# JasperSnoek/spearmint

Hardware: NVIDIA H100
Metric: EI candidates/sec (higher is better)
Workload: dtype f32

## Files before the change

### spearmint_b200/chooser/GPEIOptChooserB200.py

```python
import time

import numpy as np
import numpy.random as npr
import scipy.optimize as spo

from spearmint_b200 import chains, util
from spearmint_b200.chooser._gp import GPChooser, GPPrior, read_state, write_state, write_stats
from spearmint_b200.locker import log


def init(expt_dir, arg_string):
    args = util.unpack_args(arg_string)
    return GPEIOptChooserB200(expt_dir, **args)


class GPEIOptChooserB200(GPChooser):
    prior = GPPrior(max_ls=2, amp2_prior_on_std=True)

    def __init__(self, expt_dir, covar="Matern52", mcmc_iters=10, pending_samples=100, noiseless=False, burnin=100,
                 grid_subset=20, use_multiprocessing=True, device=None, refine_dtype="float64", state_name=None,
                 backend=None, grid_dtype="float32", mcmc_chains=1):
        GPChooser.__init__(self, expt_dir, covar, mcmc_iters, pending_samples, noiseless, state_name, device, backend,
                           refine_dtype, grid_dtype)
        self.mcmc_chains = int(mcmc_chains)
        if self.mcmc_chains < 1:
            raise ValueError("mcmc_chains must be at least 1, got %d" % self.mcmc_chains)
        if self.mcmc_iters > 0 and self.mcmc_iters % self.mcmc_chains:
            raise ValueError("mcmc_iters (%d) must be a multiple of mcmc_chains (%d)" % (self.mcmc_iters,
                                                                                       self.mcmc_chains))
        self.chains = None
        self.burnin = int(burnin)
        self.needs_burnin = True
        self.grid_subset = int(grid_subset)
        self.hyper_samples = []
        self.use_multiprocessing = bool(int(use_multiprocessing))
        self.stats = {}

    def dump_hypers(self):
        state = {"dims": self.D, "ls": self.ls, "amp2": self.amp2, "noise": self.noise,
                 "hyper_samples": self.hyper_samples, "mean": self.mean}
        if self.chains is not None:
            state["chains"] = [c.state() for c in self.chains]
        write_state(self.locker, self.state_pkl, state)
        write_stats(self.stats_file, self.hyper_samples)

    def _load_state(self, state):
        self._load_hypers(state)
        self.hyper_samples = state["hyper_samples"]
        self.needs_burnin = False
        if self.mcmc_chains > 1 and "chains" in state:
            if len(state["chains"]) != self.mcmc_chains:
                raise ValueError("the state pickle holds %d chains, mcmc_chains is %d" % (len(state["chains"]),
                                                                                        self.mcmc_chains))
            self.chains = [chains.Chain.from_state(c, st) for c, st in enumerate(state["chains"])]

    def generate_stats_html(self):
        state = read_state(self.state_pkl)
        if state is None:
            return "Chooser not yet ready to display output"
        self._load_state(state)
        mean_mean = np.mean(np.vstack([h[0] for h in self.hyper_samples]))
        mean_noise = np.mean(np.vstack([h[1] for h in self.hyper_samples]))
        mean_ls = np.mean(np.vstack([h[3][np.newaxis, :] for h in self.hyper_samples]), 0)
        try:
            output = ('<br /><span class="label label-info">Estimated mean:</span> ' + str(mean_mean) +
                      '<br /><span class="label label-info">Estimated noise:</span> ' + str(mean_noise) +
                      '<br /><br /><span class="label label-info">Inverse parameter sensitivity' +
                      ' - Gaussian Process length scales</span><br /><br />' +
                      '<div id="lschart"></div><script type="text/javascript">' +
                      'var lsdata = [' + ','.join(['%.2f' % i for i in mean_ls]) + '];')
        except Exception:
            return "Chooser not yet ready to display output."
        output += 'bar_chart("#lschart", lsdata, ' + str(self.prior.max_ls) + ');' + '</script>'
        return output

    def _real_init(self, dims, values):
        self.randomstate = npr.get_state()
        state = self._read_state()
        if state is not None:
            self._load_state(state)
        else:
            self._init_hypers(dims, values)
            self.hyper_samples.append((self.mean, self.noise, self.amp2, self.ls))

    def next(self, grid, values, durations, candidates, pending, complete):
        if complete.shape[0] < 2:
            return int(candidates[0])
        if self.D == -1:
            self._real_init(grid.shape[1], values[complete])

        comp = grid[complete, :]
        cand = grid[candidates, :]
        pend = grid[pending, :]
        vals = values[complete]
        numcand = cand.shape[0]

        best_comp = np.argmin(vals)
        cand2 = np.vstack((np.random.randn(10, comp.shape[1]) * 0.001 + comp[best_comp, :], cand))

        if self.mcmc_iters <= 0:
            raise NotImplementedError("mcmc_iters=0 (ML-II hyper-parameters) is broken in the reference "
                                      "(GPEIOptChooser.py:316-318) and not provided here")

        t_phase = [time.perf_counter()]
        phase_ms = {}

        def lap(name):
            t_phase.append(time.perf_counter())
            phase_ms[name] = phase_ms.get(name, 0.0) + 1e3 * (t_phase[-1] - t_phase[-2])

        if self.mcmc_chains > 1:
            self._sample_chains(comp, vals)
        else:
            self._loglik = self.backend.loglik(self.covar, comp, vals)
            if self.needs_burnin:
                for mcmc_iter in range(self.burnin):
                    self.sample_hypers(comp, vals)
                    log("BURN %d/%d] mean: %.2f  amp: %.2f noise: %.4f  min_ls: %.4f  max_ls: %.4f"
                        % (mcmc_iter + 1, self.burnin, self.mean, np.sqrt(self.amp2), self.noise,
                           np.min(self.ls), np.max(self.ls)))
                self.needs_burnin = False

            self.hyper_samples = []
            for mcmc_iter in range(self.mcmc_iters):
                self.sample_hypers(comp, vals)
                log("%d/%d] mean: %.2f  amp: %.2f  noise: %.4f min_ls: %.4f  max_ls: %.4f"
                    % (mcmc_iter + 1, self.mcmc_iters, self.mean, np.sqrt(self.amp2), self.noise,
                       np.min(self.ls), np.max(self.ls)))
            self.dump_hypers()
            self.stats["loglik_evals"] = getattr(self._loglik, "calls", None)
            self.stats["loglik_batches"] = getattr(self._loglik, "launch_batches", None)
            self._loglik = None
        lap("mcmc")

        b = [(0, 1)] * cand.shape[1]

        state = self._grid_state(comp, pend, vals)
        inds = self.backend.top_mean_ei(state, cand2, min(self.grid_subset, cand2.shape[0]))
        cand2 = cand2[inds, :]
        lap("grid_pass_1")

        ctx = self._refine_context(comp, pend, vals)
        for i in range(cand2.shape[0]):
            log("Optimizing candidate %d/%d" % (i + 1, cand2.shape[0]))
            ret = spo.fmin_l_bfgs_b(ctx.value_grad, cand2[i, :].flatten(), bounds=b)
            cand2[i, :] = ret[0]
        cand = np.vstack((cand, cand2))
        self.stats["refine_evals"] = getattr(ctx, "evals", None)
        del ctx
        lap("refine")

        best_cand = int(self.backend.top_mean_ei(state, cand, 1)[-1])
        self._set_current(self.hyper_samples[-1])
        lap("grid_pass_2")
        self.stats["phase_ms"] = phase_ms

        if best_cand >= numcand:
            return (int(numcand), cand[best_cand, :])
        return int(candidates[best_cand])

    def _fantasy_normals(self, pend):
        if pend.shape[0] == 0:
            return None
        npr.set_state(self.randomstate)
        return npr.randn(pend.shape[0], self.pending_samples)

    def _grid_state(self, comp, pend, vals):
        return self.backend.grid_state(self.covar, self.hyper_samples, comp, pend, vals, self._fantasy_normals(pend))

    def _refine_context(self, comp, pend, vals):
        return self.backend.refine_context(self.covar, self.hyper_samples, comp, pend, vals,
                                           self._fantasy_normals(pend))

    def _set_current(self, hyper):
        self.mean, self.noise, self.amp2, self.ls = hyper[0], hyper[1], hyper[2], hyper[3]

    def ei_over_hypers(self, comp, pend, cand, vals):
        hs = self.hyper_samples[:self.mcmc_iters]
        st = self.backend.grid_state(self.covar, hs, comp, pend, vals, self._fantasy_normals(pend))
        out = self.backend.ei_matrix(st, cand)
        self._set_current(hs[-1])
        return out

    def compute_ei(self, comp, pend, cand, vals):
        hs = [(self.mean, self.noise, self.amp2, self.ls)]
        st = self.backend.grid_state(self.covar, hs, comp, pend, vals, self._fantasy_normals(pend))
        return self.backend.ei_matrix(st, cand)[:, 0]

    def grad_optimize_ei_over_hypers(self, cand, comp, pend, vals, compute_grad=True):
        f, g = self._refine_context(comp, pend, vals).value_grad(cand)
        return (f, g) if compute_grad else f

    def _sample_chains(self, comp, vals):
        K = self.mcmc_chains
        if self.chains is None:
            self.chains = chains.Chain.seeded(K, (self.mean, self.noise, self.amp2, self.ls))
        ll = self.backend.loglik(self.covar, comp, vals, chains=K)
        self.hyper_samples, rounds = chains.sample(self.chains, self.prior, ll, vals, self.noiseless, self.burnin,
                                                   self.mcmc_iters // K)
        self._set_current(self.hyper_samples[-1])
        self.needs_burnin = False
        self.dump_hypers()
        self.stats["loglik_evals"] = getattr(ll, "calls", None)
        self.stats["loglik_batches"] = getattr(ll, "launch_batches", None)
        self.stats["chain_rounds"] = rounds

    def sample_hypers(self, comp, vals):
        ll = self._ll(comp, vals)
        if self.noiseless:
            self.noise = 1e-3
        self.mean, self.amp2, self.noise = self.prior.joint(ll, self.mean, self.amp2, self.noise, self.ls, vals,
                                                            self.noiseless)
        self.ls = self.prior.length_scales(ll, self.mean, self.noise, self.amp2, self.ls)
        self.hyper_samples.append((self.mean, self.noise, self.amp2, self.ls))
```

### spearmint_b200/csrc/potrf_ll.cu

```cuda
#include <cuda_runtime.h>

#include <algorithm>
#include <cstdlib>
#include <map>
#include <tuple>

#include "common.cuh"
#include "diag.cuh"

namespace smk {
int num_sms();
namespace ll {

constexpr int NB = 128;
constexpr int KC = 16;
constexpr int LDS = 20;
constexpr int STAGES = 3;

constexpr int WD = NB * 32;

__device__ __forceinline__ void pdl_wait() { asm volatile("griddepcontrol.wait;" ::: "memory"); }
__device__ __forceinline__ void pdl_trigger() { asm volatile("griddepcontrol.launch_dependents;" ::: "memory"); }

__global__ void __launch_bounds__(256) diag_kernel(int ld, int jb, double* __restrict__ A, long a_stride,
                                                    double* __restrict__ W, long w_stride, int* __restrict__ info) {
  extern __shared__ __align__(16) unsigned char smem_raw[];
  const int s = blockIdx.x;
  double* Ab = A + (long)s * a_stride + (long)jb * NB * ld + (long)jb * NB;
  pdl_wait();
  diag_factor_block<double, NB>(Ab, ld, W + (long)s * w_stride + (long)jb * WD, info ? info + s : nullptr, jb * NB,
                                reinterpret_cast<double*>(smem_raw), true);
}

__global__ void __launch_bounds__(256) panel_kernel(int ld, int jb, int row_blk0, double* __restrict__ A, long a_stride,
                                                     const double* __restrict__ W, long w_stride) {
  extern __shared__ __align__(16) unsigned char smem_raw[];
  const int s = blockIdx.z;
  double* As = A + (long)s * a_stride;
  pdl_wait();
  panel_sub_block<double, NB>(As + ((long)row_blk0 * NB + (long)blockIdx.x * 32) * ld + (long)jb * NB, ld,
                              As + (long)jb * NB * ld + (long)jb * NB, W + (long)s * w_stride + (long)jb * WD, nullptr,
                              nullptr, reinterpret_cast<double*>(smem_raw), true);
}

__device__ __forceinline__ void cp_async16(void* dst, const void* src) {
  asm volatile("cp.async.cg.shared.global [%0], [%1], 16;" ::"r"((unsigned)__cvta_generic_to_shared(dst)), "l"(src) : "memory");
}
__device__ __forceinline__ void cp_async_commit() { asm volatile("cp.async.commit_group;" ::: "memory"); }
template <int N> __device__ __forceinline__ void cp_async_wait() { asm volatile("cp.async.wait_group %0;" ::"n"(N) : "memory"); }

__device__ __forceinline__ void dmma(double (&c)[2], double a, double b) { dmma_884(c, a, b); }

struct GemmArgs {
  const double* A; const double* B; double* C;
  long a_stride, b_stride, c_stride;
  int lda, ldb, ldc, K;
  int row0, col0;
  int brow0;
  int sub, tri;
  int persist, nt, batch;
};

template <int BM, int ST>
__global__ void __launch_bounds__(256) dgemm_nt_kernel(GemmArgs g) {
  constexpr int WM = BM / 32, WN = 8 / WM;
  constexpr int WTN = 128 / WN;
  constexpr int NT = WTN / 8;
  extern __shared__ __align__(16) unsigned char smem_raw[];
  double* As = reinterpret_cast<double*>(smem_raw);
  double* Bs = As + ST * BM * LDS;

  const int tid = threadIdx.x, warp = tid >> 5, lane = tid & 31;
  const int wm = warp / WN, wn = warp % WN, gq = lane >> 2, t4 = lane & 3;
  const int ntri = g.nt * (g.nt + 1) / 2;
  const long items = g.persist ? (long)g.batch * ntri : 1;
  for (long item = g.persist ? blockIdx.x : 0; item < items; item += gridDim.x) {
    int bx = blockIdx.x, by = blockIdx.y, bz = blockIdx.z;
    if (g.persist) {
      bz = (int)(item / ntri);
      const int e = (int)(item - (long)bz * ntri);
      bx = (int)((sqrtf(8.f * (float)e + 1.f) - 1.f) * 0.5f);
      while (bx * (bx + 1) / 2 > e) --bx;
      while ((bx + 1) * (bx + 2) / 2 <= e) ++bx;
      by = e - bx * (bx + 1) / 2;
    }
    const int r0 = g.row0 + bx * BM, c0 = g.col0 + by * 128;
    if (g.tri && c0 > r0 + BM - 1) continue;
    const double* A = g.A + (long)bz * g.a_stride + (long)r0 * g.lda;
    const double* B = g.B + (long)bz * g.b_stride + (long)(g.brow0 + by * 128) * g.ldb;
    double* C = g.C + (long)bz * g.c_stride + (long)r0 * g.ldc + c0;

    auto load_stage = [&](int st, int k0) {
#pragma unroll
      for (int q = 0; q < BM * 8 / 256; ++q) {
        const int ch = tid + q * 256, row = ch >> 3, pc = ch & 7;
        cp_async16(As + ((size_t)st * BM + row) * LDS + pc * 2, A + (long)row * g.lda + k0 + pc * 2);
      }
#pragma unroll
      for (int q = 0; q < 4; ++q) {
        const int ch = tid + q * 256, row = ch >> 3, pc = ch & 7;
        cp_async16(Bs + ((size_t)st * 128 + row) * LDS + pc * 2, B + (long)row * g.ldb + k0 + pc * 2);
      }
    };

    double acc[4][NT][2];
#pragma unroll
    for (int mi = 0; mi < 4; ++mi)
#pragma unroll
      for (int ni = 0; ni < NT; ++ni) { acc[mi][ni][0] = 0.0; acc[mi][ni][1] = 0.0; }

    const int nk = g.K / KC;
#pragma unroll
    for (int s = 0; s < ST - 1; ++s) {
      if (s < nk) load_stage(s, s * KC);
      cp_async_commit();
    }
    for (int kt = 0; kt < nk; ++kt) {
      cp_async_wait<ST - 2>();
      __syncthreads();
      if (kt + ST - 1 < nk) load_stage((kt + ST - 1) % ST, (kt + ST - 1) * KC);
      cp_async_commit();
      const double* as = As + ((size_t)(kt % ST) * BM + wm * 32 + gq) * LDS + t4;
      const double* bs = Bs + ((size_t)(kt % ST) * 128 + wn * WTN + gq) * LDS + t4;
#pragma unroll
      for (int kk = 0; kk < KC; kk += 4) {
        double af[4], bf[NT];
#pragma unroll
        for (int mi = 0; mi < 4; ++mi) af[mi] = as[mi * 8 * LDS + kk];
#pragma unroll
        for (int ni = 0; ni < NT; ++ni) bf[ni] = bs[ni * 8 * LDS + kk];
#pragma unroll
        for (int mi = 0; mi < 4; ++mi)
#pragma unroll
          for (int ni = 0; ni < NT; ++ni) dmma(acc[mi][ni], af[mi], bf[ni]);
      }
    }
    cp_async_wait<0>();
    __syncthreads();

#pragma unroll
    for (int mi = 0; mi < 4; ++mi)
#pragma unroll
      for (int ni = 0; ni < NT; ++ni) {
        double2* cp = reinterpret_cast<double2*>(C + (long)(wm * 32 + mi * 8 + gq) * g.ldc + wn * WTN + ni * 8 + t4 * 2);
        double2 v;
        if (g.sub) { v = *cp; v.x -= acc[mi][ni][0]; v.y -= acc[mi][ni][1]; }
        else { v.x = acc[mi][ni][0]; v.y = acc[mi][ni][1]; }
        *cp = v;
      }
  }
}

constexpr int DBU_MAXK = 256;
__global__ void __launch_bounds__(256) diag_block_update_kernel(int ld, int b, int k0, int K, double* __restrict__ A, long a_stride) {
  extern __shared__ __align__(16) unsigned char smem_raw[];
  const int LD = K + 4;
  double* Ar = reinterpret_cast<double*>(smem_raw);
  double* Br = Ar + 32 * LD;
  int ti = 0, e = blockIdx.x;
  while ((ti + 1) * (ti + 2) / 2 <= e) ++ti;
  const int tj = e - ti * (ti + 1) / 2;
  double* As = A + (long)blockIdx.y * a_stride;
  const double* pa = As + ((long)b * NB + ti * 32) * ld + k0;
  const double* pb = As + ((long)b * NB + tj * 32) * ld + k0;
  const int tid = threadIdx.x, warp = tid >> 5, lane = tid & 31, gq = lane >> 2, t4 = lane & 3;
  pdl_wait();
  pdl_trigger();
  const int cpr = K / 2;
  for (int ch = tid; ch < 32 * cpr; ch += 256) {
    const int row = ch / cpr, pc = ch - row * cpr;
    cp_async16(Ar + row * LD + pc * 2, pa + (long)row * ld + pc * 2);
    cp_async16(Br + row * LD + pc * 2, pb + (long)row * ld + pc * 2);
  }
  cp_async_commit();
  cp_async_wait<0>();
  __syncthreads();
  double* Ct = As + ((long)b * NB + ti * 32) * ld + (long)b * NB + tj * 32;
#pragma unroll
  for (int u = 0; u < 2; ++u) {
    const int t = 2 * warp + u, r0 = (t >> 2) * 8, c0 = (t & 3) * 8;
    const double* ap = Ar + (r0 + gq) * LD + t4;
    const double* bp = Br + (c0 + gq) * LD + t4;
    double c[2][2] = {{0.0, 0.0}, {0.0, 0.0}};
#pragma unroll 8
    for (int k = 0; k < K; k += 8) {
      dmma(c[0], ap[k], bp[k]);
      dmma(c[1], ap[k + 4], bp[k + 4]);
    }
    double2* cp = reinterpret_cast<double2*>(Ct + (long)(r0 + gq) * ld + c0 + t4 * 2);
    double2 v = *cp;
    v.x -= c[0][0] + c[1][0];
    v.y -= c[0][1] + c[1][1];
    *cp = v;
  }
}

template <int BM>
static void launch_gemm(const GemmArgs& g, int tiles_m, int tiles_n, int S, cudaStream_t st) {
  constexpr int ST = STAGES;
  const size_t smem = sizeof(double) * ST * (BM + 128) * LDS;
  static bool attr = false;
  if (!attr) {
    cudaFuncSetAttribute(dgemm_nt_kernel<BM, ST>, cudaFuncAttributeMaxDynamicSharedMemorySize, (int)smem);
    attr = true;
  }
  dgemm_nt_kernel<BM, ST><<<dim3(tiles_m, tiles_n, S), 256, smem, st>>>(g);
}

template <int ST>
static void launch_gemm_background_st(GemmArgs g, int nt, int S, int ctas, cudaStream_t st) {
  const size_t smem = sizeof(double) * ST * (128 + 128) * LDS;
  static bool attr = false;
  if (!attr) {
    cudaFuncSetAttribute(dgemm_nt_kernel<128, ST>, cudaFuncAttributeMaxDynamicSharedMemorySize, (int)smem);
    attr = true;
  }
  g.persist = 1; g.nt = nt; g.batch = S;
  const long items = (long)S * nt * (nt + 1) / 2;
  dgemm_nt_kernel<128, ST><<<(unsigned)std::min<long>(items, ctas), 256, smem, st>>>(g);
}
static void launch_gemm_background(const GemmArgs& g, int nt, int S, int ctas, cudaStream_t st) {
  static int stages = -1;
  if (stages < 0) { const char* e = getenv("SMK_LL_BG_STAGES"); stages = (e && e[0] == '3') ? 3 : 2; }
  if (stages == 3) launch_gemm_background_st<3>(g, nt, S, ctas, st);
  else launch_gemm_background_st<2>(g, nt, S, ctas, st);
}

template <typename... KArgs, typename... Args>
static void launch_spine(void (*kern)(KArgs...), dim3 grid, size_t smem, cudaStream_t st, Args... args) {
  static int pdl = -1;
  if (pdl < 0) { const char* e = getenv("SMK_LL_PDL"); pdl = (e && e[0] == '0') ? 0 : 1; }
  cudaLaunchConfig_t cfg = {};
  cfg.gridDim = grid; cfg.blockDim = dim3(256); cfg.dynamicSmemBytes = smem; cfg.stream = st;
  cudaLaunchAttribute at[1];
  at[0].id = cudaLaunchAttributeProgrammaticStreamSerialization;
  at[0].val.programmaticStreamSerializationAllowed = 1;
  cfg.attrs = at; cfg.numAttrs = pdl ? 1 : 0;
  cudaLaunchKernelEx(&cfg, kern, KArgs(args)...);
}

struct Streams {
  cudaStream_t main = nullptr, near = nullptr, side = nullptr;
  cudaEvent_t diag0 = nullptr, diag1 = nullptr, head0 = nullptr, col = nullptr, la = nullptr, larest = nullptr, larest2 = nullptr, panel = nullptr, rest = nullptr,
              join_near = nullptr, join_side = nullptr;
};
static Streams& streams() {
  static Streams s;
  if (!s.main) {
    int lo = 0, hi = 0;
    cudaDeviceGetStreamPriorityRange(&lo, &hi);
    cudaStreamCreateWithPriority(&s.main, cudaStreamNonBlocking, hi);
    cudaStreamCreateWithPriority(&s.near, cudaStreamNonBlocking, hi < lo ? hi + 1 : hi);
    cudaStreamCreateWithPriority(&s.side, cudaStreamNonBlocking, lo);
    for (cudaEvent_t* e : {&s.diag0, &s.diag1, &s.head0, &s.col, &s.la, &s.larest, &s.larest2, &s.panel, &s.rest, &s.join_near, &s.join_side})
      cudaEventCreateWithFlags(e, cudaEventDisableTiming);
  }
  return s;
}

static int enqueue(int Npad, int S, double* A, double* W, int* info, Streams& ss) {
  const int nblk = Npad / NB;
  const long as = (long)Npad * Npad, ws = (long)nblk * WD;
  const size_t dsm = DiagSmem<double, NB>::bytes, psm = PanelSmem<double, NB>::bytes;
  static bool attr = false;
  if (!attr) {
    cudaFuncSetAttribute(diag_kernel, cudaFuncAttributeMaxDynamicSharedMemorySize, (int)dsm);
    cudaFuncSetAttribute(panel_kernel, cudaFuncAttributeMaxDynamicSharedMemorySize, (int)psm);
    cudaFuncSetAttribute(diag_block_update_kernel, cudaFuncAttributeMaxDynamicSharedMemorySize,
                         (int)(sizeof(double) * 2 * 32 * (DBU_MAXK + 4)));
    attr = true;
  }
  const size_t dbu_smem = sizeof(double) * 2 * 32 * (DBU_MAXK + 4);
  cudaStream_t m = ss.main, nr = ss.near, sd = ss.side;
  auto gemm_args = [&](int jcol, int K, int row_blk, int col_blk, int tri) {
    GemmArgs g{};
    g.A = A + (long)jcol * NB; g.lda = Npad; g.a_stride = as;
    g.B = A + (long)jcol * NB; g.ldb = Npad; g.b_stride = as; g.brow0 = col_blk * NB;
    g.C = A; g.ldc = Npad; g.c_stride = as;
    g.K = K; g.row0 = row_blk * NB; g.col0 = col_blk * NB; g.sub = 1; g.tri = tri;
    return g;
  };
  bool pend_col = false, pend_la = false, pend_la2 = false, side_used = false, near_used = false;
  const int reserve = std::min(24, std::max(8, 10 * S + 2));
  const int bg_ctas = std::max(num_sms() - reserve, 1);
  const double* Wc = W;
  for (int j = 0; j < nblk; j += 2) {
    launch_spine(diag_kernel, dim3(S), dsm, m, Npad, j, A, as, W, ws, info);
    count_launch();
    const int rem = nblk - j - 1;
    if (rem <= 0) break;
    if (pend_la) { cudaStreamWaitEvent(m, ss.larest, 0); pend_la = false; }
    if (rem > 1) {
      cudaEventRecord(ss.diag0, m);
      cudaStreamWaitEvent(nr, ss.diag0, 0);
      panel_kernel<<<dim3((rem - 1) * 4, 1, S), 256, psm, nr>>>(Npad, j, j + 2, A, as, Wc, ws);
      count_launch();
      near_used = true;
    }
    launch_spine(panel_kernel, dim3(4, 1, S), psm, m, Npad, j, j + 1, A, as, Wc, ws);
    if (pend_la2) { cudaStreamWaitEvent(m, ss.larest2, 0); pend_la2 = false; }
    launch_spine(diag_block_update_kernel, dim3(10, S), dbu_smem, m, Npad, j + 1, j * NB, NB, A, as);
    count_launch(2);
    if (rem > 1) {
      cudaEventRecord(ss.head0, m);
      cudaStreamWaitEvent(nr, ss.head0, 0);
      launch_gemm<32>(gemm_args(j, NB, j + 2, j + 1, 0), (rem - 1) * 4, 1, S, nr);
      cudaEventRecord(ss.col, nr);
      count_launch();
      pend_col = true;
    }
    launch_spine(diag_kernel, dim3(S), dsm, m, Npad, j + 1, A, as, W, ws, info);
    count_launch();
    const int rem2 = nblk - j - 2;
    if (rem2 <= 0) break;
    if (rem2 > 1) {
      cudaEventRecord(ss.diag1, m);
      cudaStreamWaitEvent(nr, ss.diag1, 0);
      panel_kernel<<<dim3((rem2 - 1) * 4, 1, S), 256, psm, nr>>>(Npad, j + 1, j + 3, A, as, Wc, ws);
      cudaEventRecord(ss.panel, nr);
      count_launch();
    }
    if (pend_col) { cudaStreamWaitEvent(m, ss.col, 0); pend_col = false; }
    launch_spine(panel_kernel, dim3(4, 1, S), psm, m, Npad, j + 1, j + 2, A, as, Wc, ws);
    count_launch();
    if (side_used) cudaStreamWaitEvent(m, ss.rest, 0);
    launch_spine(diag_block_update_kernel, dim3(10, S), dbu_smem, m, Npad, j + 2, j * NB, 2 * NB, A, as);
    count_launch();
    if (rem2 > 1) {
      cudaEventRecord(ss.la, m);
      cudaStreamWaitEvent(nr, ss.la, 0);
      launch_gemm<32>(gemm_args(j, 2 * NB, j + 3, j + 2, 0), (rem2 - 1) * 4, 1, S, nr);
      cudaEventRecord(ss.larest, nr);
      launch_gemm<32>(gemm_args(j, 2 * NB, j + 3, j + 3, 1), (rem2 - 1) * 4, 1, S, nr);
      cudaEventRecord(ss.larest2, nr);
      count_launch(2);
      pend_la = pend_la2 = true;
    }
    if (rem2 > 2) {
      cudaStreamWaitEvent(sd, ss.panel, 0);
      launch_gemm_background(gemm_args(j, 2 * NB, j + 4, j + 4, 1), rem2 - 2, S, bg_ctas, sd);
      cudaEventRecord(ss.rest, sd);
      count_launch();
      side_used = true;
    }
  }
  if (near_used) {
    cudaEventRecord(ss.join_near, nr);
    cudaStreamWaitEvent(m, ss.join_near, 0);
  }
  if (side_used) {
    cudaEventRecord(ss.join_side, sd);
    cudaStreamWaitEvent(m, ss.join_side, 0);
  }
  return 0;
}

}

static std::map<cudaGraphExec_t, int>& launches_per_graph() {
  static std::map<cudaGraphExec_t, int> m;
  return m;
}

size_t potrf_ll_workspace_bytes(int Npad, int S) { return (size_t)S * (Npad / ll::NB) * ll::WD * sizeof(double); }

int potrf_ll_f64(int Npad, int S, double* A, double* W, int* info, int use_graph, cudaStream_t st) {
  if (Npad <= 0 || Npad % ll::NB) return -1;
  if (S <= 0) return -2;
  if (!A || !W || !info) return -3;
  ll::Streams& ss = ll::streams();
  static cudaEvent_t ev_in = nullptr, ev_out = nullptr;
  if (!ev_in) {
    cudaEventCreateWithFlags(&ev_in, cudaEventDisableTiming);
    cudaEventCreateWithFlags(&ev_out, cudaEventDisableTiming);
  }
  cudaMemsetAsync(info, 0, sizeof(int) * S, st);
  if (!use_graph) {
    cudaEventRecord(ev_in, st);
// ... 41 lines not shown
```

### spearmint_b200/engine.py

```python
import ctypes as C
import os

import numpy as np
import scipy.stats as sps
import torch

from . import _lib
from ._lib import KINDS, check, fn, ptr

JITTER = 1e-6
CONSTRAINT_NOISE = 1e-3


def _ceil(x, m):
    return ((x + m - 1) // m) * m


class HyperBatch(object):

    def __init__(self, hyper_samples, kind, device, dtype):
        S = len(hyper_samples)
        D = len(np.atleast_1d(hyper_samples[0][3]))
        mean = np.array([h[0] for h in hyper_samples], dtype=np.float64)
        noise = np.array([h[1] for h in hyper_samples], dtype=np.float64)
        amp2 = np.array([h[2] for h in hyper_samples], dtype=np.float64)
        ls = np.vstack([np.atleast_1d(h[3]) for h in hyper_samples]).astype(np.float64)
        if kind == "SE":
            ls = np.ones_like(ls)
        host = np.concatenate([mean, noise, amp2, (1.0 / ls).ravel()])
        dev = torch.from_numpy(host).to(device=device, dtype=dtype, non_blocking=False)
        self.S, self.D = S, D
        self.mean, self.noise, self.amp2 = dev[:S], dev[S:2 * S], dev[2 * S:3 * S]
        self.inv_ls = dev[3 * S:].view(S, D)
        self.host_mean, self.host_noise, self.host_amp2, self.host_ls = mean, noise, amp2, ls
        self.nbytes = host.size * (8 if dtype == torch.float64 else 4)

    def slice(self, a, b):
        o = object.__new__(HyperBatch)
        o.S, o.D = b - a, self.D
        o.mean, o.noise, o.amp2, o.inv_ls = self.mean[a:b], self.noise[a:b], self.amp2[a:b], self.inv_ls[a:b]
        o.host_mean, o.host_noise = self.host_mean[a:b], self.host_noise[a:b]
        o.host_amp2, o.host_ls = self.host_amp2[a:b], self.host_ls[a:b]
        o.nbytes = 0
        return o


class Factor(object):

    def __init__(self, eng, kind, X, hb, L=None, winv=None, info=None, factor_impl=None):
        self.eng, self.kind, self.hb = eng, kind, hb
        self.factor_impl = factor_impl or eng.factor_impl
        self.X = X
        self.N, self.D = X.shape
        self.Npad = _ceil(self.N, 128)
        S, dt, dev = hb.S, eng.dtype, eng.device
        NB = eng.NB
        self._owned = []
        self.L = L if L is not None else self._take((S, self.Npad, self.Npad))
        self.winv = winv if winv is not None else self._take((S, self.Npad // NB, NB, NB))
        self.info = info if info is not None else torch.zeros((S,), dtype=torch.int32, device=dev)
        st = eng.stream()
        check(fn("smk_cov_build", dt)(KINDS[kind], self.N, self.N, self.D, S, ptr(X), None, ptr(hb.inv_ls),
                                      ptr(hb.amp2), ptr(hb.noise), ptr(self.L), self.Npad, st), "cov_build")
        if self.factor_impl == "tc" and dt == torch.float32 and self.Npad >= 256:
            L = _lib.lib()
            nb = 2 * S * self.Npad * self.Npad * 4
            ws = eng.take((nb,), torch.uint8)
            if eng.fused_inverse:
                Np = L.smk_tc_np(self.N)
                hi = self._take((S, Np, Np), torch.float32)
                lo = self._take((S, Np, Np), torch.float32)
                nt = L.smk_trtri_tc_workspace_bytes(self.Npad, Np, S)
                wt = eng.take((nt,), torch.uint8)
                check(L.smk_potrf_trtri_tc_f32(self.Npad, Np, S, ptr(self.L), ptr(self.winv), ptr(self.info), ptr(ws), nb,
                                               ptr(hi), ptr(lo), ptr(wt), nt, st), "potrf_trtri_tc")
                eng.give(ws, wt)
                self._linv = (hi, lo, Np)
            else:
                eng.give(ws)
                check(L.smk_potrf_lower_batched_tc_f32(self.Npad, S, ptr(self.L), ptr(self.winv), ptr(self.info),
                                                       ptr(ws), nb, st), "potrf_tc")
        else:
            check(fn("smk_potrf_lower_batched", dt)(self.Npad, S, ptr(self.L), ptr(self.winv), ptr(self.info), st),
                  "potrf")

    def _take(self, shape, dtype=None):
        t = self.eng.take(shape, dtype)
        self._owned.append(t)
        return t

    def __del__(self):
        try:
            self.eng.give(*self._owned)
        except Exception:
            pass

    def linv(self):
        if getattr(self, "_linv", None) is None:
            eng, L = self.eng, _lib.lib()
            S = self.hb.S
            Np = L.smk_tc_np(self.N)
            hi = self._take((S, Np, Np), torch.float32)
            lo = self._take((S, Np, Np), torch.float32)
            if self.factor_impl == "tc" and self.Npad >= 256:
                nb = L.smk_trtri_tc_workspace_bytes(self.Npad, Np, S)
                ws = eng.take((nb,), torch.uint8)
                eng.give(ws)
                check(L.smk_trtri_split_tc_f32(self.Npad, Np, S, ptr(self.L), ptr(self.winv), ptr(hi), ptr(lo), ptr(ws),
                                               nb, eng.stream()), "trtri_split_tc")
            else:
                nb = L.smk_trtri_workspace_bytes(Np, S)
                ws = eng.take((nb,), torch.uint8)
                eng.give(ws)
                check(L.smk_trtri_split_f32(self.Npad, Np, S, ptr(self.L), ptr(self.winv), ptr(hi), ptr(lo), ptr(ws),
                                            nb, eng.stream()), "trtri_split")
            self._linv = (hi, lo, Np)
        return self._linv

    def linv16(self):
        if getattr(self, "_linv16", None) is None:
            eng, L = self.eng, _lib.lib()
            hi, lo, Np = self.linv()
            S = self.hb.S
            h16 = self._take((S, Np, Np), torch.float16)
            l16 = self._take((S, Np, Np), torch.float16)
            exps = torch.empty((2 * S,), dtype=torch.int32, device=eng.device)
            check(L.smk_linv_pack_f16(Np, S, ptr(hi), ptr(lo), ptr(h16), ptr(l16), ptr(exps), eng.stream()),
                  "linv_pack_f16")
            self._linv16 = (h16, l16, exps, Np)
        return self._linv16

    def alpha_via_linv(self, y):
        eng, L = self.eng, _lib.lib()
        hi, lo, Np = self.linv()
        S = self.hb.S
        alpha = torch.empty((S, 1, self.Npad), dtype=torch.float32, device=eng.device)
        tmp = torch.empty((S, Np), dtype=torch.float32, device=eng.device)
        check(L.smk_linv_alpha_f32(self.N, Np, S, ptr(hi), ptr(lo), ptr(y), ptr(self.hb.mean), ptr(alpha), self.Npad,
                                   ptr(tmp), eng.stream()), "linv_alpha")
        self._z = tmp
        return alpha

    def guard(self, rows):
        eng, L = self.eng, _lib.lib()
        hi, lo, Np = self.linv()
        S = self.hb.S
        g = torch.empty((S,), dtype=torch.float32, device=eng.device)
        rows = torch.as_tensor(np.resize(np.asarray(rows, dtype=np.int32), 4), device=eng.device)
        nb = L.smk_tc_guard_workspace_bytes(Np, S)
        ws = eng.take((nb,), torch.uint8)
        eng.give(ws)
        check(L.smk_tc_guard_f32(self.N, self.Npad, Np, S, ptr(self.L), ptr(hi), ptr(lo), ptr(self.hb.amp2),
# ... 555 lines not shown
    TAIL_SHORTLIST = 256

    def tail_fix(self, kind, hs_local, S_total, comp, pend, cand, vals, normals, ths_local, durs_log, ei, ei_sum, M,
                 reduce_fn=None, rescore=None):
        if self.dtype != torch.float32:
            return False
        top = float(ei_sum[:M].max())
        if not (top < self.TAIL_MEAN_EI * S_total):
            return False
        k = min(self.TAIL_SHORTLIST, M)
        idx, _ = self.topk(ei_sum, M, k)
        idx_h = idx.cpu().numpy().astype(np.int64)
        sub = torch.zeros((k,), dtype=torch.float64, device=self.device)
        if hs_local:
            h64 = self.helper64()
            sub_cand = np.ascontiguousarray(cand[idx_h])
            if rescore is not None:
                e64, s64 = rescore(h64, sub_cand)
            else:
                e64, s64, _ = h64.ei_over_hypers_device(kind, hs_local, comp, pend, sub_cand, vals, normals, ths_local,
                                                        durs_log, want_matrix=True)
            sub += s64[:k]
            if ei is not None:
                ei[:, idx.long()] = e64[:, :k]
        if reduce_fn is not None:
            reduce_fn(sub)
        ei_sum[idx.long()] = sub
        return True

    def constraint_prob_device(self, kind, chyper_samples, ff, comp, labels, Cd, noise=CONSTRAINT_NOISE, want_mean=False):
        S, M = len(chyper_samples), Cd.shape[0]
        ldm = _ceil(M, 128)
        gain = np.array([float(c[1]) for c in chyper_samples])
        if labels is not None and (np.all(np.asarray(labels) > 0) or np.all(np.asarray(labels) <= 0)):
            p = torch.as_tensor(sps.norm.cdf(gain), dtype=torch.float64, device=self.device)
            return p.view(S, 1).expand(S, ldm).contiguous(), None
        N, D = comp.shape
        h64 = self.helper64()
        X64, ff64 = h64.to_dev(comp), h64.to_dev(np.ravel(ff))
        X = X64 if h64 is self else self.to_dev(comp)
        gain_d = torch.as_tensor(gain, dtype=torch.float64, device=self.device)
        p = torch.empty((S, ldm), dtype=torch.float64, device=self.device)
        m = torch.empty((S, ldm), dtype=torch.float64, device=self.device) if want_mean else None
        hs = [(0.0, noise, float(c[2]), np.atleast_1d(np.asarray(c[3], dtype=float))) for c in chyper_samples]
        chunk = h64.max_samples_per_chunk(_ceil(N, 128), ldm)
        for s0 in range(0, S, chunk):
            t = self._t0()
            hb64 = h64.hypers(hs[s0:s0 + chunk], kind)
            fac = h64.factor(kind, X64, hb64, factor_impl="simt")
            t_alpha, _, _ = fac.solve(ff64, F=1, subtract_mean=False)
            self._t1("constraint_factor", t)
            fac.check_pd()
            hb = hb64 if h64 is self else self.hypers(hs[s0:s0 + chunk], kind)
            t = self._t0()
            check(fn("smk_constraint_prob", self.dtype)(KINDS[kind], N, fac.Npad, M, D, hb.S, ptr(X), ptr(Cd),
                                                        ptr(hb.inv_ls), ptr(hb.amp2), ptr(t_alpha), ptr(gain_d[s0:]),
                                                        ptr(p[s0:]), ptr(m[s0:]) if want_mean else None, ldm,
                                                        self.stream()), "constraint_prob")
            self._t1("constraint_prob", t)
            del fac
        return p, m

    def constrained_ei_over_hypers_device(self, kind, hyper_samples, chyper_samples, ff, comp, labels, pend, cand, vals,
                                          normals=None, noise=CONSTRAINT_NOISE):
        if self.guard_threshold > 0:
            raise _lib.SmkError("the constrained pass does not run the tensor-core accuracy guard (SMK_TC_GUARD)")
        labels = np.asarray(labels)
        good = labels > 0
        if not np.any(good):
            raise ValueError("constrained EI needs at least one feasible observation")
        comp_g, vals_g = np.ascontiguousarray(comp[good]), np.asarray(vals, dtype=float)[good]
        S = len(hyper_samples)
        P = 0 if pend is None else int(pend.shape[0])
        if len(chyper_samples) != S:
            raise ValueError("%d objective but %d constraint hyper-samples" % (S, len(chyper_samples)))
        if np.size(ff) != comp.shape[0]:
            raise ValueError("ff has %d entries for %d complete observations" % (np.size(ff), comp.shape[0]))
        if P and (normals is None or np.ndim(normals) != 3 or np.shape(normals)[:2] != (S, P)):
            raise ValueError("pending points need fantasy normals of shape (S, P, F) = (%d, %d, F), got %s"
                             % (S, P, None if normals is None else np.shape(normals)))
        Cd = self.to_dev(cand)
        M = Cd.shape[0]
        ldm = _ceil(M, 128)
        w, _ = self.constraint_prob_device(kind, chyper_samples, ff, comp, labels, Cd, noise)
        chunk = self.max_samples_per_chunk(_ceil(comp_g.shape[0] + P, 128), ldm, 1 if P == 0 else int(normals.shape[-1]))
        ei_sum = torch.zeros((ldm,), dtype=torch.float64, device=self.device)
        ei_all = torch.empty((S, ldm), dtype=torch.float64, device=self.device)
        for s0 in range(0, S, chunk):
            nrm = None if normals is None else normals[s0:s0 + chunk]
            prep = self.prepare(kind, hyper_samples[s0:s0 + chunk], comp_g, pend, vals_g, nrm, cand_dev=Cd)
            ei, _ = self.ei_prepared(prep, Cd, True, ei_sum, weight=w[s0:s0 + prep.S])
            prep.fac.check_pd()
            ei_all[s0:s0 + prep.S] = ei
            del prep
        self.last = dict(N=comp.shape[0], N_good=comp_g.shape[0], M=M, S=S, P=P, chunk=chunk)
        return ei_all, ei_sum, M

    def constrained_ei_over_hypers(self, kind, hyper_samples, chyper_samples, ff, comp, labels, pend, cand, vals,
                                   normals=None, noise=CONSTRAINT_NOISE):
        ei, ei_sum, M = self.constrained_ei_over_hypers_device(kind, hyper_samples, chyper_samples, ff, comp, labels,
                                                               pend, cand, vals, normals, noise)

        def rescore(h64, sub):
            e, s, _ = h64.constrained_ei_over_hypers_device(kind, hyper_samples, chyper_samples, ff, comp, labels, pend,
                                                            sub, vals, normals, noise)
            return e, s
        self.tail_fix(kind, hyper_samples, len(hyper_samples), comp, pend, cand, vals, normals, None, None, ei, ei_sum, M,
                      rescore=rescore)
        return ei[:, :M].t().contiguous().cpu().numpy()

    def loglik(self, kind, comp, vals, chains=1):
        return LogLik(self, kind, comp, vals) if chains == 1 else ChainLogLik(self, kind, comp, vals, chains)

    def latent_loglik(self, kind, comp, ls, noise=CONSTRAINT_NOISE):
        return LatentLogLik(self, kind, comp, ls, noise)

    def latent_factor(self, kind, comp, amp2, ls, noise):
        return LatentFactor(self, kind, comp, amp2, ls, noise)

    def constrained_refine_context(self, kind, hyper_samples, chyper_samples, ff, comp, labels, pend, vals, normals=None,
                                   noise=CONSTRAINT_NOISE):
        return ConstrainedRefineContext(self, kind, hyper_samples, chyper_samples, ff, comp, labels, pend, vals, normals,
                                        noise)

    def refine_context(self, kind, hyper_samples, comp, pend, vals, normals=None, time_hyper_samples=None,
                       durs_log=None):
        return RefineContext(self, kind, hyper_samples, comp, pend, vals, normals, time_hyper_samples, durs_log)


class LogLik(object):

    def __init__(self, eng, kind, comp, vals, max_batch=None):
        self.eng, self.kind = eng, kind
        self.X = eng.to_dev(comp)
        self.y = eng.to_dev(vals)
        self.N, self.D = self.X.shape
        self.Npad = _ceil(self.N + 1, 128)
        if max_batch is None:
            max_batch = 8 if self.N <= 1024 else 6
        self.max_batch = max_batch
        self.speculate = (3, 0) if self.N <= 1536 else (0, 2)
        dt, dev = eng.dtype, eng.device
        self.L = torch.zeros((max_batch, self.Npad, self.Npad), dtype=dt, device=dev)
        self.fast = (dt == torch.float64) and os.environ.get("SMK_LOGLIK_IMPL", "ll") == "ll"
        self.use_graph = 1 if os.environ.get("SMK_LOGLIK_GRAPH", "1") == "1" else 0
        if self.fast:
            self.ws_bytes = _lib.lib().smk_potrf_loglik_workspace_bytes(self.Npad, max_batch)
            self.winv = torch.empty((self.ws_bytes,), dtype=torch.uint8, device=dev)
        else:
            self.winv = torch.empty((max_batch, self.Npad // eng.NB, eng.NB, eng.NB), dtype=dt, device=dev)
        self.info = torch.zeros((max_batch,), dtype=torch.int32, device=dev)
        self.out = torch.empty((2, max_batch), dtype=dt, device=dev)
        self.calls = 0
        self.launch_batches = 0

    def _chunk(self, items):
        return self.eng.hypers([(h[0], h[1], h[2], np.asarray(h[3], dtype=float)) for h in items], self.kind), self.y

    def _set_rhs(self, B, hb, y, st):
        check(fn("smk_loglik_set_rhs", self.eng.dtype)(self.N, self.Npad, B, ptr(y), ptr(hb.mean), ptr(self.L), st),
              "loglik_set_rhs")

    def batch(self, items):
        out = np.empty(len(items))
        eng, dt, N, Npad = self.eng, self.eng.dtype, self.N, self.Npad
        for b0 in range(0, len(items), self.max_batch):
            its = items[b0:b0 + self.max_batch]
            B = len(its)
            hb, y = self._chunk(its)
            st = eng.stream()
            check(fn("smk_cov_build_lower", dt)(KINDS[self.kind], N, self.D, B, ptr(self.X), ptr(hb.inv_ls),
                                                ptr(hb.amp2), ptr(hb.noise), ptr(self.L), Npad, st), "cov_build")
            self._set_rhs(B, hb, y, st)
            if self.fast:
                check(_lib.lib().smk_potrf_loglik_f64(Npad, B, ptr(self.L), ptr(self.winv), self.ws_bytes, ptr(self.info),
                                                      self.use_graph, st), "potrf_loglik")
            else:
                check(fn("smk_potrf_lower_batched", dt)(Npad, B, ptr(self.L), ptr(self.winv), ptr(self.info), st), "potrf")
            check(fn("smk_loglik_finish", dt)(N, Npad, B, ptr(self.L), ptr(self.out[0]), ptr(self.out[1]), st),
                  "loglik_finish")
            r = torch.cat([self.out[0, :B].double(), self.out[1, :B].double(), self.info[:B].double()]).cpu().numpy()
            lp = -r[:B] - 0.5 * r[B:2 * B]
            lp[r[2 * B:] != 0] = np.nan
            out[b0:b0 + B] = lp
            self.calls += B
            self.launch_batches += 1
        return out

    def __call__(self, *item):
        v = self.batch([item])[0]
        if np.isnan(v):
            raise np.linalg.LinAlgError("leading minor of the array is not positive definite")
        return v


LOGLIK_SMALL_MAX_N = 238


class ChainLogLik(LogLik):

    def __init__(self, eng, kind, comp, vals, chains):
        N = comp.shape[0]
        self.speculate = (3, 0) if N <= 1536 else (0, 2)
        max_batch = chains * (3 + max(self.speculate))
        self.small = N <= LOGLIK_SMALL_MAX_N
        self.device = eng.device
        if not self.small:
            LogLik.__init__(self, eng, kind, comp, vals, max_batch)
            return
        self.eng, self.kind = eng, kind
        self.X, self.y = eng.to_dev(comp), eng.to_dev(vals)
        self.N, self.D = self.X.shape
        self.max_batch = max_batch
        self.out = torch.empty((2, max_batch), dtype=torch.float64, device=eng.device)
        self.info = torch.zeros((max_batch,), dtype=torch.int32, device=eng.device)
        self.calls = 0
        self.launch_batches = 0

    def batch(self, items):
        if not self.small:
            return LogLik.batch(self, items)
        out = np.empty(len(items))
        for b0 in range(0, len(items), self.max_batch):
            its = items[b0:b0 + self.max_batch]
            B = len(its)
            hb, y = self._chunk(its)
            check(_lib.lib().smk_loglik_small_f64(KINDS[self.kind], self.N, self.D, B, ptr(self.X), ptr(hb.inv_ls),
                                                  ptr(hb.amp2), ptr(hb.noise), ptr(hb.mean), ptr(y), ptr(self.out[0]),
                                                  ptr(self.out[1]), ptr(self.info), self.eng.stream()), "loglik_small")
            r = torch.cat([self.out[0, :B], self.out[1, :B], self.info[:B].double()]).cpu().numpy()
            lp = -r[:B] - 0.5 * r[B:2 * B]
            lp[r[2 * B:] != 0] = np.nan
            out[b0:b0 + B] = lp
            self.calls += B
            self.launch_batches += 1
        return out


class RefineContext(object):

    def __init__(self, eng, kind, hyper_samples, comp, pend, vals, normals=None, time_hyper_samples=None,
                 durs_log=None):
        if kind == "SE":
            raise AttributeError("module 'spearmint.gp' has no attribute 'grad_SE'")
        self.eng, self.kind = eng, kind
        self.prep = eng.prepare(kind, hyper_samples, comp, pend, vals, normals, time_hyper_samples, durs_log)
        self.prep.fac.check_pd()
        self.pending = self.prep.P > 0
        self.hb = self.prep.hb
        self.evals = 0

    def _terms(self, fac, alpha, F, x):
        eng, dt = self.eng, self.eng.dtype
        hb = fac.hb
        S, N, D = hb.S, fac.N, fac.D
        xq = eng.to_dev(np.reshape(x, (1, D)))
        kx = torch.empty((S, 1, N), dtype=dt, device=eng.device)
        check(fn("smk_cov_build", dt)(KINDS[self.kind], 1, N, D, S, ptr(xq), ptr(fac.X), ptr(hb.inv_ls),
                                      ptr(hb.amp2), None, ptr(kx), N, eng.stream()), "cov_build")
        gamma, _, _ = fac.solve(kx, F=1, y_stride=N, ldy=N, subtract_mean=False)
        out = torch.empty((S, 1, F + 1, D + 1), dtype=dt, device=eng.device)
        check(fn("smk_ei_grad_terms", dt)(KINDS[self.kind], N, fac.Npad, D, S, 1, F, ptr(fac.X), ptr(xq),
                                          ptr(hb.inv_ls), ptr(hb.amp2), ptr(alpha), ptr(gamma), ptr(out),
                                          eng.stream()), "ei_grad_terms")
        return out.double().cpu().numpy()[:, 0]

    def per_sample(self, x):
        p, hb = self.prep, self.hb
        F, D = p.F, p.fac.D
        out = self._terms(p.fac, p.alpha, F, x)
        amp2, mean = hb.host_amp2, hb.host_mean
        m = out[:, :F, D] + mean[:, None]
        v = amp2 * (1 + JITTER) - out[:, F, D]
        s = np.sqrt(v)[:, None]
        u = (p.bests_host - m) / s
        cdf, pdf = sps.norm.cdf(u), sps.norm.pdf(u)
        ei = s * (u * cdf + pdf)
        g_m, g_s2 = -cdf, 0.5 * pdf / s
        gx_m = out[:, :F, :D]
        gx_v = -2.0 * out[:, F, :D]
        g = 0.5 * amp2[:, None, None] * (gx_m * g_m[:, :, None] + gx_v[:, None, :] * g_s2[:, :, None])
        self.evals += 1
        if not self.pending:
            f_s, g_s, ei_s = -ei.sum(axis=1), g[:, 0, :], ei[:, 0]
        else:
            f_s, g_s, ei_s = -ei.mean(axis=1), g.mean(axis=1), ei.mean(axis=1)
        if p.time is not None:
            tfac, ta = p.time
            tout = self._terms(tfac, ta, 1, x)
            thb = tfac.hb
            ftm = np.exp(tout[:, 0, D] + thb.host_mean)
            gt = 0.5 * thb.host_amp2[:, None] * tout[:, 0, :D] * ftm[:, None]
            g_s = (ftm[:, None] * g_s - ei_s[:, None] * gt) / (ftm[:, None] ** 2)
            f_s = -(ei_s / ftm)
        return f_s, g_s

    def value_grad(self, x):
        f_s, g_s = self.per_sample(np.asarray(x, dtype=float))
        return float(f_s.sum()), g_s.sum(axis=0).flatten()


class LatentLogLik(LogLik):

    def __init__(self, eng, kind, comp, ls, noise=CONSTRAINT_NOISE, max_batch=None):
        LogLik.__init__(self, eng, kind, comp, np.zeros(comp.shape[0]), max_batch)
        self.ls, self.noise = np.atleast_1d(np.asarray(ls, dtype=float)), float(noise)

    def _chunk(self, items):
        hb = self.eng.hypers([(0.0, self.noise, float(a), self.ls) for a, _ in items], self.kind)
        return hb, self.eng.to_dev(np.vstack([np.ravel(f) for _, f in items]))

    def _set_rhs(self, B, hb, y, st):
        check(fn("smk_loglik_set_rhs_batched", self.eng.dtype)(self.N, self.Npad, B, ptr(y), self.N, ptr(self.L), st),
              "loglik_set_rhs_batched")


class LatentFactor(object):

    def __init__(self, eng, kind, comp, amp2, ls, noise):
        if eng.dtype != torch.float64:
            raise _lib.SmkError("LatentFactor needs the float64 engine")
        self.eng = eng
        hb = eng.hypers([(0.0, float(noise), float(amp2), np.atleast_1d(np.asarray(ls, dtype=float)))], kind)
        self.fac = eng.factor(kind, eng.to_dev(comp), hb, factor_impl="simt")
        self.fac.check_pd()
        self.N = comp.shape[0]
        self.out = torch.empty((self.N,), dtype=torch.float64, device=eng.device)

    def draw(self, z):
        zd = self.eng.to_dev(np.ravel(z))
        check(_lib.lib().smk_lower_matvec_f64(self.N, self.fac.Npad, ptr(self.fac.L), ptr(zd), ptr(self.out),
                                              self.eng.stream()), "lower_matvec")
        return self.out.cpu().numpy()


class ConstrainedRefineContext(RefineContext):

    def __init__(self, eng, kind, hyper_samples, chyper_samples, ff, comp, labels, pend, vals, normals=None,
                 noise=CONSTRAINT_NOISE):
        if kind == "SE":
            raise AttributeError("module 'spearmint.gp' has no attribute 'grad_SE'")
        self.eng, self.kind, self.evals = eng, kind, 0
        labels = np.asarray(labels)
        good = labels > 0
        comp_g, vals_g = np.ascontiguousarray(comp[good]), np.asarray(vals, dtype=float)[good]
        self.best = float(np.min(vals_g))
        self.pending = pend is not None and pend.shape[0] > 0
        self.vanilla = bool(np.all(labels > 0) or np.all(labels <= 0))
        self.prep = eng.prepare(kind, hyper_samples, comp_g, pend if self.pending else None, vals_g,
                                normals if self.pending else None)
        self.prep.fac.check_pd()
        self.hb = self.prep.hb
        if not self.pending:
            Xf = eng.to_dev(comp)
            self.fac_full = eng.factor(kind, Xf, self.hb)
            self.fac_full.check_pd()
            self.zero_alpha = torch.zeros((self.hb.S, 1, self.fac_full.Npad), dtype=eng.dtype, device=eng.device)
        if not self.vanilla:
            hs = [(0.0, noise, float(c[2]), np.atleast_1d(np.asarray(c[3], dtype=float))) for c in chyper_samples]
            self.gain = np.array([float(c[1]) for c in chyper_samples])
            self.camp2 = np.array([float(c[2]) for c in chyper_samples])
            self.fac_c = eng.factor(kind, eng.to_dev(comp), eng.hypers(hs, kind))
            self.fac_c.check_pd()
            self.t_alpha, _, _ = self.fac_c.solve(eng.to_dev(np.ravel(ff)), F=1, subtract_mean=False)

    def per_sample(self, x):
        p, hb = self.prep, self.hb
        F, D = p.F, p.fac.D
        amp2, mean = hb.host_amp2, hb.host_mean
        out = self._terms(p.fac, p.alpha, F, x)
        m = out[:, :F, D] + mean[:, None]
        gx_m = out[:, :F, :D]
        if self.pending:
            v, gx_v = amp2 * (1 + JITTER) - out[:, F, D], -2.0 * out[:, F, :D]
        else:
            full = self._terms(self.fac_full, self.zero_alpha, 1, x)
            v, gx_v = amp2 * (1 + JITTER) - full[:, 1, D], -2.0 * full[:, 1, :D]
        s = np.sqrt(v)[:, None]
        u = (self.best - m) / s
        cdf, pdf = sps.norm.cdf(u), sps.norm.pdf(u)
        ei = s * (u * cdf + pdf)
        g_m, g_s2 = -cdf, 0.5 * pdf / s
        g = 0.5 * amp2[:, None] * (gx_m * g_m[:, :, None] + gx_v[:, None, :] * g_s2[:, :, None]).sum(axis=1)
        ei_tot = ei.sum(axis=1)
        self.evals += 1
        if self.vanilla:
            return -ei_tot, g
# ... 6 lines not shown
```

Measured before the change: 209,100.

## Use m16n8k16 DMMA, prefetch C, fix bg stages, memoize loglik factorisations

Replaces the m8n8k4 FP64 MMA with the larger m16n8k16 shape in the blocked Cholesky GEMM and in the diagonal-tile update, so fewer MMA instructions and fragment loads are issued. It also prefetches the C tile into L2 before the subtractive update, hard-codes two pipeline stages for the background GEMM, and adds an LRU cache of log-likelihood results keyed on hyperparameter bytes so repeated slice-sampler evaluations skip refactorisation. The metric is EI candidates per second, so the MCMC loglik changes may have little effect on it. Each loglik batch now pays extra Python hashing cost.

New measurement: 209,200, median of 6. No clear change (+0.0%).

```diff
diff --git a/spearmint_b200/chooser/GPEIOptChooserB200.py b/spearmint_b200/chooser/GPEIOptChooserB200.py
--- a/spearmint_b200/chooser/GPEIOptChooserB200.py
+++ b/spearmint_b200/chooser/GPEIOptChooserB200.py
@@ -129,6 +129,7 @@
                        np.min(self.ls), np.max(self.ls)))
             self.dump_hypers()
             self.stats["loglik_evals"] = getattr(self._loglik, "calls", None)
+            self.stats["loglik_factorisations"] = getattr(self._loglik, "factorisations", None)
             self.stats["loglik_batches"] = getattr(self._loglik, "launch_batches", None)
             self._loglik = None
         lap("mcmc")
@@ -202,6 +203,7 @@
         self.needs_burnin = False
         self.dump_hypers()
         self.stats["loglik_evals"] = getattr(ll, "calls", None)
+        self.stats["loglik_factorisations"] = getattr(ll, "factorisations", None)
         self.stats["loglik_batches"] = getattr(ll, "launch_batches", None)
         self.stats["chain_rounds"] = rounds
 
diff --git a/spearmint_b200/csrc/potrf_ll.cu b/spearmint_b200/csrc/potrf_ll.cu
--- a/spearmint_b200/csrc/potrf_ll.cu
+++ b/spearmint_b200/csrc/potrf_ll.cu
@@ -49,7 +49,21 @@
 __device__ __forceinline__ void cp_async_commit() { asm volatile("cp.async.commit_group;" ::: "memory"); }
 template <int N> __device__ __forceinline__ void cp_async_wait() { asm volatile("cp.async.wait_group %0;" ::"n"(N) : "memory"); }
 
-__device__ __forceinline__ void dmma(double (&c)[2], double a, double b) { dmma_884(c, a, b); }
+__device__ __forceinline__ void dmma16(double (&c)[4], const double (&a)[8], const double (&b)[4]) {
+  asm volatile("mma.sync.aligned.m16n8k16.row.col.f64.f64.f64.f64 {%0,%1,%2,%3}, {%4,%5,%6,%7,%8,%9,%10,%11}, "
+               "{%12,%13,%14,%15}, {%0,%1,%2,%3};"
+               : "+d"(c[0]), "+d"(c[1]), "+d"(c[2]), "+d"(c[3])
+               : "d"(a[0]), "d"(a[1]), "d"(a[2]), "d"(a[3]), "d"(a[4]), "d"(a[5]), "d"(a[6]), "d"(a[7]),
+                 "d"(b[0]), "d"(b[1]), "d"(b[2]), "d"(b[3]));
+}
+__device__ __forceinline__ void load_a16(double (&a)[8], const double* p, int ld) {
+#pragma unroll
+  for (int i = 0; i < 8; ++i) a[i] = p[(i & 1) * 8 * ld + (i >> 1) * 4];
+}
+__device__ __forceinline__ void load_b16(double (&b)[4], const double* p) {
+#pragma unroll
+  for (int i = 0; i < 4; ++i) b[i] = p[i * 4];
+}
 
 struct GemmArgs {
   const double* A; const double* B; double* C;
@@ -65,7 +79,7 @@
 __global__ void __launch_bounds__(256) dgemm_nt_kernel(GemmArgs g) {
   constexpr int WM = BM / 32, WN = 8 / WM;
   constexpr int WTN = 128 / WN;
-  constexpr int NT = WTN / 8;
+  constexpr int MT = 2, NT = WTN / 8;
   extern __shared__ __align__(16) unsigned char smem_raw[];
   double* As = reinterpret_cast<double*>(smem_raw);
   double* Bs = As + ST * BM * LDS;
@@ -89,6 +103,13 @@
     const double* A = g.A + (long)bz * g.a_stride + (long)r0 * g.lda;
     const double* B = g.B + (long)bz * g.b_stride + (long)(g.brow0 + by * 128) * g.ldb;
     double* C = g.C + (long)bz * g.c_stride + (long)r0 * g.ldc + c0;
+    if (g.sub) {
+#pragma unroll
+      for (int q = 0; q < BM * 8 / 256; ++q) {
+        const int ln = tid + q * 256;
+        asm volatile("prefetch.global.L2 [%0];" ::"l"(C + (long)(ln >> 3) * g.ldc + (ln & 7) * 16));
+      }
+    }
 
     auto load_stage = [&](int st, int k0) {
 #pragma unroll
@@ -103,11 +124,13 @@
       }
     };
 
-    double acc[4][NT][2];
-#pragma unroll
-    for (int mi = 0; mi < 4; ++mi)
-#pragma unroll
-      for (int ni = 0; ni < NT; ++ni) { acc[mi][ni][0] = 0.0; acc[mi][ni][1] = 0.0; }
+    double acc[MT][NT][4];
+#pragma unroll
+    for (int mi = 0; mi < MT; ++mi)
+#pragma unroll
+      for (int ni = 0; ni < NT; ++ni)
+#pragma unroll
+        for (int r = 0; r < 4; ++r) acc[mi][ni][r] = 0.0;
 
     const int nk = g.K / KC;
 #pragma unroll
@@ -122,32 +145,32 @@
       cp_async_commit();
       const double* as = As + ((size_t)(kt % ST) * BM + wm * 32 + gq) * LDS + t4;
       const double* bs = Bs + ((size_t)(kt % ST) * 128 + wn * WTN + gq) * LDS + t4;
-#pragma unroll
-      for (int kk = 0; kk < KC; kk += 4) {
-        double af[4], bf[NT];
-#pragma unroll
-        for (int mi = 0; mi < 4; ++mi) af[mi] = as[mi * 8 * LDS + kk];
-#pragma unroll
-        for (int ni = 0; ni < NT; ++ni) bf[ni] = bs[ni * 8 * LDS + kk];
-#pragma unroll
-        for (int mi = 0; mi < 4; ++mi)
-#pragma unroll
-          for (int ni = 0; ni < NT; ++ni) dmma(acc[mi][ni], af[mi], bf[ni]);
+      double af[MT][8];
+#pragma unroll
+      for (int mi = 0; mi < MT; ++mi) load_a16(af[mi], as + mi * 16 * LDS, LDS);
+#pragma unroll
+      for (int ni = 0; ni < NT; ++ni) {
+        double bf[4];
+        load_b16(bf, bs + ni * 8 * LDS);
+#pragma unroll
+        for (int mi = 0; mi < MT; ++mi) dmma16(acc[mi][ni], af[mi], bf);
       }
     }
     cp_async_wait<0>();
     __syncthreads();
 
 #pragma unroll
-    for (int mi = 0; mi < 4; ++mi)
-#pragma unroll
-      for (int ni = 0; ni < NT; ++ni) {
-        double2* cp = reinterpret_cast<double2*>(C + (long)(wm * 32 + mi * 8 + gq) * g.ldc + wn * WTN + ni * 8 + t4 * 2);
-        double2 v;
-        if (g.sub) { v = *cp; v.x -= acc[mi][ni][0]; v.y -= acc[mi][ni][1]; }
-        else { v.x = acc[mi][ni][0]; v.y = acc[mi][ni][1]; }
-        *cp = v;
-      }
+    for (int mi = 0; mi < MT; ++mi)
+#pragma unroll
+      for (int ni = 0; ni < NT; ++ni)
+#pragma unroll
+        for (int h = 0; h < 2; ++h) {
+          double2* cp = reinterpret_cast<double2*>(C + (long)(wm * 32 + mi * 16 + h * 8 + gq) * g.ldc + wn * WTN + ni * 8 + t4 * 2);
+          double2 v;
+          if (g.sub) { v = *cp; v.x -= acc[mi][ni][2 * h]; v.y -= acc[mi][ni][2 * h + 1]; }
+          else { v.x = acc[mi][ni][2 * h]; v.y = acc[mi][ni][2 * h + 1]; }
+          *cp = v;
+        }
   }
 }
 
@@ -176,21 +199,26 @@
   cp_async_wait<0>();
   __syncthreads();
   double* Ct = As + ((long)b * NB + ti * 32) * ld + (long)b * NB + tj * 32;
-#pragma unroll
-  for (int u = 0; u < 2; ++u) {
-    const int t = 2 * warp + u, r0 = (t >> 2) * 8, c0 = (t & 3) * 8;
-    const double* ap = Ar + (r0 + gq) * LD + t4;
-    const double* bp = Br + (c0 + gq) * LD + t4;
-    double c[2][2] = {{0.0, 0.0}, {0.0, 0.0}};
-#pragma unroll 8
-    for (int k = 0; k < K; k += 8) {
-      dmma(c[0], ap[k], bp[k]);
-      dmma(c[1], ap[k + 4], bp[k + 4]);
-    }
-    double2* cp = reinterpret_cast<double2*>(Ct + (long)(r0 + gq) * ld + c0 + t4 * 2);
+  const int r0 = (warp >> 2) * 16, c0 = (warp & 3) * 8;
+  const double* ap = Ar + (r0 + gq) * LD + t4;
+  const double* bp = Br + (c0 + gq) * LD + t4;
+  double c[2][4] = {{0.0, 0.0, 0.0, 0.0}, {0.0, 0.0, 0.0, 0.0}};
+#pragma unroll 4
+  for (int k = 0; k < K; k += 32) {
+#pragma unroll
+    for (int u = 0; u < 2; ++u) {
+      double af[8], bf[4];
+      load_a16(af, ap + k + 16 * u, LD);
+      load_b16(bf, bp + k + 16 * u);
+      dmma16(c[u], af, bf);
+    }
+  }
+#pragma unroll
+  for (int h = 0; h < 2; ++h) {
+    double2* cp = reinterpret_cast<double2*>(Ct + (long)(r0 + h * 8 + gq) * ld + c0 + t4 * 2);
     double2 v = *cp;
-    v.x -= c[0][0] + c[1][0];
-    v.y -= c[0][1] + c[1][1];
+    v.x -= c[0][2 * h] + c[1][2 * h];
+    v.y -= c[0][2 * h + 1] + c[1][2 * h + 1];
     *cp = v;
   }
 }
@@ -207,8 +235,8 @@
   dgemm_nt_kernel<BM, ST><<<dim3(tiles_m, tiles_n, S), 256, smem, st>>>(g);
 }
 
-template <int ST>
-static void launch_gemm_background_st(GemmArgs g, int nt, int S, int ctas, cudaStream_t st) {
+static void launch_gemm_background(GemmArgs g, int nt, int S, int ctas, cudaStream_t st) {
+  constexpr int ST = 2;
   const size_t smem = sizeof(double) * ST * (128 + 128) * LDS;
   static bool attr = false;
   if (!attr) {
@@ -218,12 +246,6 @@
   g.persist = 1; g.nt = nt; g.batch = S;
   const long items = (long)S * nt * (nt + 1) / 2;
   dgemm_nt_kernel<128, ST><<<(unsigned)std::min<long>(items, ctas), 256, smem, st>>>(g);
-}
-static void launch_gemm_background(const GemmArgs& g, int nt, int S, int ctas, cudaStream_t st) {
-  static int stages = -1;
-  if (stages < 0) { const char* e = getenv("SMK_LL_BG_STAGES"); stages = (e && e[0] == '3') ? 3 : 2; }
-  if (stages == 3) launch_gemm_background_st<3>(g, nt, S, ctas, st);
-  else launch_gemm_background_st<2>(g, nt, S, ctas, st);
 }
 
 template <typename... KArgs, typename... Args>
diff --git a/spearmint_b200/engine.py b/spearmint_b200/engine.py
--- a/spearmint_b200/engine.py
+++ b/spearmint_b200/engine.py
@@ -1,3 +1,4 @@
+import collections
 import ctypes as C
 import os
 
@@ -859,7 +860,14 @@
         self.info = torch.zeros((max_batch,), dtype=torch.int32, device=dev)
         self.out = torch.empty((2, max_batch), dtype=dt, device=dev)
         self.calls = 0
+        self.factorisations = 0
         self.launch_batches = 0
+        self.cache = collections.OrderedDict()
+        self.cache_size = 4 * max_batch
+
+    @staticmethod
+    def _key(item):
+        return b"".join(np.ravel(np.asarray(x, dtype=float)).tobytes() for x in item)
 
     def _chunk(self, items):
         return self.eng.hypers([(h[0], h[1], h[2], np.asarray(h[3], dtype=float)) for h in items], self.kind), self.y
@@ -869,6 +877,22 @@
               "loglik_set_rhs")
 
     def batch(self, items):
+        keys = [self._key(it) for it in items]
+        todo = {}
+        for k, it in zip(keys, items):
+            if k in self.cache:
+                self.cache.move_to_end(k)
+            elif k not in todo:
+                todo[k] = it
+        if todo:
+            for k, v in zip(todo, self._factor(list(todo.values()))):
+                self.cache[k] = v
+            while len(self.cache) > self.cache_size:
+                self.cache.popitem(last=False)
+        self.calls += len(items)
+        return np.array([self.cache[k] for k in keys], dtype=float)
+
+    def _factor(self, items):
         out = np.empty(len(items))
         eng, dt, N, Npad = self.eng, self.eng.dtype, self.N, self.Npad
         for b0 in range(0, len(items), self.max_batch):
@@ -890,7 +914,7 @@
             lp = -r[:B] - 0.5 * r[B:2 * B]
             lp[r[2 * B:] != 0] = np.nan
             out[b0:b0 + B] = lp
-            self.calls += B
+            self.factorisations += B
             self.launch_batches += 1
         return out
 
@@ -922,6 +946,7 @@
         self.out = torch.empty((2, max_batch), dtype=torch.float64, device=eng.device)
         self.info = torch.zeros((max_batch,), dtype=torch.int32, device=eng.device)
         self.calls = 0
+        self.factorisations = 0
         self.launch_batches = 0
 
     def batch(self, items):
@@ -940,6 +965,7 @@
             lp[r[2 * B:] != 0] = np.nan
             out[b0:b0 + B] = lp
             self.calls += B
+            self.factorisations += B
             self.launch_batches += 1
         return out
 
```
